# AnnSeidel/genometools

Hardware: AMD Instinct MI355X
Metric: Gbp/s ESA build (suf+lcp+bwt), 3 Gbp DNA, 1/2/4/8 MI355X; bit-exact vs CPU (higher is better)
Workload: dtype u64; 1 GPU; human-like DNA (2% N, 24 seqs, repeats) n=3000000000 seed=43 -suf -lcp -bwt (BASELINE.json configs[2]); parallelism=1 device, pair_suffixes=341032298, tied_suffixes=390540711, refine_rounds=9, maxbranchdepth=8256

## Files before the change

### genometools_amd/csrc/esa_engine.hip

```cpp
#include <stdarg.h>
#include <stdlib.h>
#include <chrono>
#include <type_traits>
#include <utility>
#include <vector>
#include "../../include/gtamd_esa.h"
#include "esa_prims.h"
#include "esa_devutil.h"
#include "esa_own.h"

static thread_local char g_err[1024] = "";
void gtamd_set_error(const char *fmt, ...) {
  va_list ap;
  va_start(ap, fmt);
  vsnprintf(g_err, sizeof g_err, fmt, ap);
  va_end(ap);
}
extern "C" const char *gtamd_esa_last_error(void) { return g_err; }

extern "C" int gtamd_device_count(void) {
  GTAMD_ABI_BEGIN
  int n = 0;
  if (hipGetDeviceCount(&n) != hipSuccess) return 0;
  return n;
// ... 2434 lines not shown
    return e != nullptr && e[0] == c;
  };
  if (const char *e = getenv("GTAMD_MSD")) sw.msd = e[0] == '1';
  sw.msd_part_off = flag("GTAMD_MSD", '0');
  if (const char *e = getenv("GTAMD_MSD_CBITS")) {
    const int v = atoi(e);
    if (v >= 0 && v <= 8) sw.msd_cbits = v;
  }
  if (const char *e = getenv("GTAMD_MSD_BIG_MAX")) {
    const long v = atol(e);
    if (v >= MS_TILE && v <= (long) MSD_BIG_MAX) sw.msd_big_max = (u32) v;
  }
  sw.msd_radix = flag("GTAMD_MSD_RADIX", '1');
  if (const char *e = getenv("GTAMD_MSD_PACK")) sw.msd_pack = atoi(e) != 0;
  if (const char *e = getenv("GTAMD_MSD_PACK_CAP")) {
    const long v = atol(e);
    if (v >= 1024 && v <= (long) MD_CAP) sw.msd_pack_cap = (u32) v;
  }
  if (const char *e = getenv("GTAMD_MSD_BIN_LIMIT")) {
    const long v = atol(e);
    if (v >= 2 && v <= 4096) sw.msd_bin_limit = (u32) v;
  }
  sw.fused_pass0 = !flag("GTAMD_FUSED_PASS0", '0');
  sw.force_wide = flag("GTAMD_FORCE_WIDE", '1');
  sw.no_pairs = flag("GTAMD_NO_PAIRS", '1');
  sw.no_small_groups = flag("GTAMD_NO_SMALL_GROUPS", '1');
  if (const char *e = getenv("GTAMD_APPLY_EARLY")) sw.apply_early = atoi(e);
  if (sw.apply_early < 0 || sw.apply_early > 2) sw.apply_early = 0;
  if (const char *e = getenv("GTAMD_APPLY_WGS")) {
    const long v = atol(e);
    if (v >= 64 && v <= (1 << 22)) sw.apply_wgs = (u64) v;
    sw.apply_wgs_given = true;
  }
  if (const char *e = getenv("GTAMD_RANK_WINDOW_BITS")) {
    const int v = atoi(e);
    if (v >= 2 && v <= RW_BITS) sw.rank_window_bits = v;
  }
  sw.rank_all_windows = flag("GTAMD_RANK_ALL_WINDOWS", '1');
  sw.win_filter_global = flag("GTAMD_WIN_FILTER_LDS", '0');
  if (const char *e = getenv("GTAMD_PAIR_CHUNK")) {
    const int v = atoi(e);
    if (v >= 4 && v <= 1024) sw.pair_chunk = v;
  }
  if (const char *e = getenv("GTAMD_ROUND_STRIDE")) {
    const int v = atoi(e);
    if (v >= RT_STRIDE_MIN && v <= RT_TILE) sw.round_stride = (u32) v;
  }
  sw.debug = getenv("GTAMD_DEBUG") != nullptr;
  return sw;
}

struct gtamd_esa_ctx {
  int device = 0;
  u32 sigma = 0;
  int bits = 0;
  u64 max_n = 0, n = 0, N = 0;
  int readmode = 0;
  Stream st, st2;
  Event ev_sorted, ev_emitted, ev_applied;
  DevBuf tb_own, sp_own;
  Text text = {};
  bool have_text = false;
  DevBuf k0, k1, v0, v1;
  DevBuf isa_tmp;
  DevBuf rws;
  DevBuf msd;
  DevBuf suf, lcp, bwt;
  DevBuf tiebits, tiebits2;
  DevBuf arena;
  DevBuf arena_p;
  DevBuf xrecv;
  DevBuf winbuf;
  DevBuf lcpfull_buf;
  DevBuf partws;
  DevBuf posw;
  Dev<u64> llv;
  u64 llv_pairs = 0;
  Dev<u32> bck;
  u64 bck_codes = 0, bck_special = 0, bck_dist = 0;
  Dev<Stats> d_stats;
  Pinned<Stats> h_stats;
  Pinned<u32> h_counts;
  Pinned<u32> h_hist;
  u32 user_prefixlength = 0;
  u32 part = 0, numparts = 1;
  gtamd_allgather_fn comm_allgather = nullptr;
  gtamd_alltoallv_fn comm_alltoallv = nullptr;
  void (*comm_abort)(void *) = nullptr;
  void *comm_abort_user = nullptr;
  void *comm_user = nullptr;
  u64 NL = 0, index_offset = 0;
  Dev<u32> d_parthist;
  Dev<u8> d_owner;
  Dev<u32> d_counts;
  u32 want = 0;
  bool ran = false;
  gtamd_esa_stats stats = {};
  gtamd_esa_timing timing = {};
  u64 alloc_bytes = 0;
  float alloc_ms = 0;
  Event ev[8];
  Event ev_scatter[2 * 16];
};

enum TimingEvent {
  EV_START,
  EV_KEYS,
  EV_SORTED,
  EV_TIEBITS,
  EV_REFINE_BEGIN,
  EV_REFINE_END,
  EV_DONE
};

static int ensure_buf(gtamd_esa_ctx *c, DevBuf &b, u64 bytes, const char *what) {
  if (bytes <= b.bytes) return 0;
  HIP_TRY(hipStreamSynchronize(c->st));
  HIP_TRY(hipStreamSynchronize(c->st2));
  const auto t0 = std::chrono::steady_clock::now();
  c->alloc_bytes -= b.bytes;
  b.reset();
  bytes = (bytes + 255) & ~255ull;
  const hipError_t me = b.alloc(bytes);
  c->alloc_ms += std::chrono::duration<float, std::milli>(std::chrono::steady_clock::now() - t0).count();
  if (me != hipSuccess) {
    (void) hipGetLastError();
    size_t mfree = 0, mtotal = 0;
    (void) hipMemGetInfo(&mfree, &mtotal);
    gtamd_set_error("cannot allocate %llu bytes of device memory for %s: the "
                    "context holds %llu bytes already, %llu of the device's %llu "
                    "are free",
                    (unsigned long long) bytes, what,
                    (unsigned long long) c->alloc_bytes, (unsigned long long) mfree,
                    (unsigned long long) mtotal);
    return -1;
  }
  c->alloc_bytes += bytes;
  return 0;
}

extern "C" void gtamd_esa_destroy(gtamd_esa_ctx *c) {
  if (c == nullptr) return;
  (void) hipSetDevice(c->device);
  if (c->st != nullptr) (void) hipStreamSynchronize(c->st);
  if (c->st2 != nullptr) (void) hipStreamSynchronize(c->st2);
  delete c;
}

static u64 max_positions(int bits) {
  const int spare = bits == 2 ? Key<2>::SPARE_BITS : Key<5>::SPARE_BITS;
  const int total = 32 + spare > 40 ? 40 : 32 + spare;
  return 1ull << total;
}

static int create_resources(gtamd_esa_ctx *c) {
  HIP_TRY(hipSetDevice(c->device));
  HIP_TRY(create(c->st, hipStreamNonBlocking));
  HIP_TRY(create(c->st2, hipStreamNonBlocking));
  HIP_TRY(create(c->ev_sorted, hipEventDisableTiming));
  HIP_TRY(create(c->ev_emitted, hipEventDisableTiming));
  HIP_TRY(create(c->ev_applied, hipEventDisableTiming));
  HIP_TRY(c->d_stats.alloc(sizeof(Stats)));
  HIP_TRY(c->h_stats.alloc(sizeof(Stats)));
  HIP_TRY(c->h_counts.alloc(4 * DEST_MAXPARTS * 4));
  HIP_TRY(c->h_hist.alloc(PART_BINS * 4));
  HIP_TRY(c->d_parthist.alloc(PART_BINS * 4));
  HIP_TRY(c->d_owner.alloc(PART_BINS));
  HIP_TRY(c->d_counts.alloc(4 * DEST_MAXPARTS * 4));
  for (Event &e : c->ev) HIP_TRY(create(e));
  for (Event &e : c->ev_scatter) HIP_TRY(create(e));
  return 0;
}

extern "C" gtamd_esa_ctx *gtamd_esa_create(int device, uint64_t max_n,
                                           uint32_t numofchars) {
  GTAMD_ABI_BEGIN
  if (gtamd_device_count() <= device || device < 0) {
    gtamd_set_error("no HIP device %d available (this library has no CPU "
                    "fallback)", device);
    return nullptr;
  }
  if (numofchars < 2 || numofchars > 28) {
    gtamd_set_error("alphabet size %u not supported (2..28)", numofchars);
    return nullptr;
  }
  const int bits = numofchars <= 4 ? 2 : 5;
  if (max_n + 1 >= max_positions(bits) - 4096) {
    gtamd_set_error("sequence of %llu symbols exceeds the position range of "
                    "this engine (%llu)", (unsigned long long) max_n,
                    (unsigned long long) max_positions(bits));
    return nullptr;
  }
  gtamd_esa_ctx *c = new gtamd_esa_ctx();
  c->device = device;
  c->sigma = numofchars;
// ... 243 lines not shown
  return 0;
}
template <typename F>
static int dest_place(gtamd_esa_ctx *c, const F &f, u64 m, const u8 *dest, const u32 *boff) {
  if (m == 0) return 0;
  const u64 nb = div_up(m, 256);
  k_dest_place<F><<<(u32) nb, 256, 0, c->st>>>(f, m, c->numparts, nb, dest, boff);
  HIP_TRY(hipGetLastError());
  return 0;
}
static u64 dest_words(u32 R, u64 m) { return (u64) R * div_up(m ? m : 1, 256) + 16; }

template <int BITS>
static int build_bcktab(gtamd_esa_ctx *c, const u64 *skey, const u32 *spos, u64 NL, u32 k,
                        hipStream_t st) {
  u64 codes = 1, special = 1, dist = 0, pw = 1;
  for (u32 j = 0; j < k; j++) {
    if (codes > (1ull << 31) / c->sigma) {
      gtamd_set_error("bucket table for prefixlength %u over %u letters is too "
                      "large", k, c->sigma);
      return -1;
    }
    codes *= c->sigma;
  }
  for (u32 j = 0; j + 1 < k; j++) special *= c->sigma;
  for (u32 j = 1; j + 1 < k; j++) { pw *= c->sigma; dist += pw; }
  const u64 total = codes + 1 + special + dist;
  HIP_TRY(c->bck.alloc(total * 4));
  HIP_TRY(hipMemsetAsync(c->bck, 0, total * 4, st));
  if (NL > 0) {
    k_bck_count<BITS><<<(u32) div_up(NL, 256), 256, 0, st>>>(
        skey, NL, k, c->sigma, c->bck, c->bck + codes + 1,
        c->bck + codes + 1 + special, c->text, spos);
    HIP_TRY(hipGetLastError());
  }
  u32 *ws = c->rws.as<u32>();
  Dev<u32> own;
  if (scan_workspace_words(codes + 1) * 4 > c->rws.bytes) {
    HIP_TRY(own.alloc(scan_workspace_words(codes + 1) * 4));
    ws = own;
  }
  TRY(scan_u32(SCAN_SUM, c->bck, c->bck, codes + 1, false, ws, st));
  c->bck_codes = codes; c->bck_special = special; c->bck_dist = dist;
  return 0;
}

static u64 rws_words_for(u64 cap) {
  return radix_workspace_words(cap) + 10 * (div_up(cap, 64) + 64) +
         scan_workspace_words(div_up(cap, 64)) + 64;
}
static int ensure_workspace(gtamd_esa_ctx *c, u64 cap, u32 want, bool dist) {
  const u64 pad = cap + 8;
  TRY(ensure_buf(c, c->k0, pad * 8, "sort keys"));
  TRY(ensure_buf(c, c->k1, pad * 8, "sort keys"));
  TRY(ensure_buf(c, c->v0, pad * 4, "sort values"));
  TRY(ensure_buf(c, c->v1, pad * 4, "sort values"));
  TRY(ensure_buf(c, c->rws, rws_words_for(cap) * 4, "the radix workspace"));
  TRY(ensure_buf(c, c->tiebits, (div_up(cap, 64) + 2) * 8, "the tie bitmap"));
  if (want & GTAMD_WANT_SUF) TRY(ensure_buf(c, c->suf, pad * 8, "the suffix table"));
  if (want & GTAMD_WANT_LCP) TRY(ensure_buf(c, c->lcp, pad, "the lcp table"));
  if (want & GTAMD_WANT_BWT) TRY(ensure_buf(c, c->bwt, pad, "the bwt table"));
  if (dist) TRY(ensure_buf(c, c->isa_tmp, pad * 8, "the exchange scratch"));
  return 0;
}

static int msd_cbits_max(u64 N) {
  const int c = bits_for(N > 1 ? N - 1 : 1) - 24;
  return c < 0 ? 0 : (c > 8 ? 8 : c);
}
static int msd_choose_cbits(u64 N, int cmax, const float *penalty) {
  int best = cmax;
  float best_cost = 0.0f;
  for (int k = 1; k >= 0; k--) {
    const int c = cmax - 2 + k;
    if (c < 6) continue;
    const float gain = k == 1 ? 0.17f : 0.57f;
    const float cost = (penalty[k] - penalty[2]) / (float) N - gain;
    if (cost < best_cost) { best = c; best_cost = cost; }
  }
  return best;
}
struct MsdWs {
  u32 *hist, *scanws, *tcnt, *tfirst, *dtcnt, *dtfirst, *startA, *startB, *F, *scan2, *counters,
      *biglist, *giantlist, *crowdlist, *bndA;
  MsTile *desc;
  MdTile *dtiles;
  u64 *firstkey, *lastkey;
  u32 rows, tilesB_ub, tilesC_ub, tilesD_ub;
  u64 nf;
};
static u64 msd_carve(u64 N, int cb, u8 *base, MsdWs *w) {
  const u32 ntA = (u32) div_up(N, MS_TILE);
  w->tilesB_ub = ntA + 256;
  w->tilesC_ub = ntA + MSD_PARENTS;
  w->tilesD_ub = (u32) (2 * div_up(N, MS_TILE)) + MSD_PARENTS + 8;
  w->rows = w->tilesC_ub + 2;
  w->nf = (u64) MSD_PARENTS << cb;
  Bump b;
  b.base = base;
  b.off = 0;
  w->hist = b.take<u32>((u64) w->rows * 256);
  w->scanws = b.take<u32>(radix_rows_workspace_words(w->rows));
  w->desc = b.take<MsTile>(w->tilesC_ub);
  w->tcnt = b.take<u32>(MSD_PARENTS + 8);
  w->tfirst = b.take<u32>(MSD_PARENTS + 8);
  w->dtcnt = b.take<u32>(MSD_PARENTS + 8);
  w->dtfirst = b.take<u32>(MSD_PARENTS + 8);
  w->startA = b.take<u32>(256 + 8);
  w->bndA = b.take<u32>(256 * MSD_BLOCKS);
  w->startB = b.take<u32>(MSD_PARENTS + 8);
  w->F = b.take<u32>(w->nf + 8);
  w->scan2 = b.take<u32>(scan_workspace_words(w->nf + 1) + 64);
  w->counters = b.take<u32>(16);
  w->dtiles = b.take<MdTile>(w->tilesD_ub);
  w->firstkey = b.take<u64>(w->tilesD_ub);
  w->lastkey = b.take<u64>(w->tilesD_ub);
  w->biglist = b.take<u32>(w->tilesD_ub);
  w->crowdlist = b.take<u32>(w->tilesD_ub);
  w->giantlist = b.take<u32>((u64) (N / MS_TILE) + 8);
  return b.off + 256;
}

static int msd_level_prepare(gtamd_esa_ctx *c, const MsdWs &w, const u32 *pstart, u32 np, int cb,
                             u32 tiles_ub, const u32 *kin, const u64 *ein, u32 *cstart) {
  hipStream_t st = c->st;
  k_msd_tilecount<<<(np + 1 + 255) / 256, 256, 0, st>>>(pstart, 0, np, (u32) MS_TILE, w.tcnt);
  HIP_TRY(hipGetLastError());
  TRY(scan_u32(SCAN_SUM, w.tcnt, w.tfirst, (u64) np + 1, false, w.scan2, st));
  k_msd_tiledesc<<<(tiles_ub + 255) / 256, 256, 0, st>>>(pstart, w.tfirst, np, tiles_ub, w.desc);
  HIP_TRY(hipGetLastError());
  if (ein != nullptr)
    k_msd_hist_lvl<u64><<<tiles_ub + 1, MS_THREADS, 0, st>>>(ein, w.desc, tiles_ub, 32 - cb, w.hist);
  else
    k_msd_hist_lvl<u32><<<tiles_ub + 1, MS_THREADS, 0, st>>>(kin, w.desc, tiles_ub, 32 - cb, w.hist);
  HIP_TRY(hipGetLastError());
  TRY(radix_scan_tile_rows(w.hist, tiles_ub + 1, w.scanws, st));
  const u64 nchild = (u64) np << cb;
  k_msd_tot<<<(u32) div_up(nchild + 1, 256), 256, 0, st>>>(w.hist, w.tfirst, np, cb, cstart);
  HIP_TRY(hipGetLastError());
  TRY(scan_u32(SCAN_SUM, cstart, cstart, nchild + 1, false, w.scan2, st));
  return 0;
}

struct MsdPartSrc {
  const u64 *ck;
  const u32 *cp32;
  u64 index_offset;
  const unsigned long long *prev_key;
  int has_prev;
};
template <int FMT>
static int msd_sort_emit(gtamd_esa_ctx *c, const Switches &sw, u32 want, u32 prefixlength, u64 N,
                         u64 density_n, const MsdPartSrc *src, u32 **sa_out,
                         u64 **fkey, u32 **fval, u64 *local_entries) {
  hipStream_t st = c->st;
  const int cmax = msd_cbits_max(density_n);
  int cb = sw.msd_cbits >= 0 ? sw.msd_cbits : cmax;
  MsdWs w;
  const u64 bytes = msd_carve(N, cb > cmax ? cb : cmax, nullptr, &w);
  TRY(ensure_buf(c, c->msd, bytes, "the tables of the first sort"));
  (void) msd_carve(N, cb > cmax ? cb : cmax, c->msd.as<u8>(), &w);
  const u32 ntA = (u32) div_up(N, MS_TILE);
  const u32 last_valid = (u32) (N - (u64) (ntA - 1) * MS_TILE);
  const u64 pad = N + 8;
  u32 *ka = c->k0.as<u32>(), *pa = c->v0.as<u32>();
  u32 *kb = c->k1.as<u32>(), *pb = c->v1.as<u32>();
  u8 *xa = c->k1.as<u8>() + pad * 4;
  u64 *ea = c->k0.as<u64>();
  const bool wide = src == nullptr;
  const int lbits = msd_block_bits(N);
  if (src != nullptr)
    k_msd_hist_a_keys<<<ntA, MS_THREADS, 0, st>>>(src->ck, N, w.hist);
  else if (FMT == 1)
    k_msd_hist_a5<<<ntA, MS_THREADS, 0, st>>>(c->text, N, w.hist);
  else
    k_msd_hist_a<<<ntA, MS_THREADS, 0, st>>>(c->text, N, w.hist);
  HIP_TRY(hipGetLastError());
  TRY(radix_scan_tile_rows(w.hist, ntA, w.scanws, st));
  k_msd_starts_a<<<wide ? MSD_BLOCKS : 1, 256, 0, st>>>(w.hist, (u32) N, ntA, lbits, w.startA,
                                                         wide ? w.bndA : nullptr);
  HIP_TRY(hipGetLastError());
  if (src != nullptr)
    k_msd_scatter_a<1><<<((ntA + 7u) >> 3) * 8u, MS_THREADS, 0, st>>>(
        c->text, N, last_valid, w.hist, ntA, src->ck, src->cp32, ka, xa, pa, nullptr);
  else if (FMT == 1)
    k_msd_scatter_a<2><<<((ntA + 7u) >> 3) * 8u, MS_THREADS, 0, st>>>(
        c->text, N, last_valid, w.hist, ntA, nullptr, nullptr, nullptr, nullptr, nullptr, ea);
  else
    k_msd_scatter_a<0><<<((ntA + 7u) >> 3) * 8u, MS_THREADS, 0, st>>>(
        c->text, N, last_valid, w.hist, ntA, nullptr, nullptr, nullptr, nullptr, nullptr, ea);
  HIP_TRY(hipGetLastError());
  HIP_TRY(hipEventRecord(c->ev[EV_KEYS], st));
  TRY(msd_level_prepare(c, w, w.startA, 256, 8, w.tilesB_ub, ka, wide ? ea : nullptr, w.startB));
  if (wide)
    k_msd_scatter_lvl<1, true><<<((w.tilesB_ub + 7u) >> 3) * 8u, MS_THREADS, 0, st>>>(
        nullptr, nullptr, nullptr, ea, w.bndA, lbits, w.desc, w.tilesB_ub, w.hist, w.tfirst,
        w.startB, 8, 24, kb, pb);
  else
    k_msd_scatter_lvl<1, false><<<((w.tilesB_ub + 7u) >> 3) * 8u, MS_THREADS, 0, st>>>(
        ka, xa, pa, nullptr, nullptr, 0, w.desc, w.tilesB_ub, w.hist, w.tfirst, w.startB, 8, 24,
        kb, pb);
  HIP_TRY(hipGetLastError());
  if (sw.msd_cbits < 0 && cmax >= 1) {
    float *d_exp = reinterpret_cast<float *>(w.counters);
    float *h_exp = c->h_counts.as<float>();
    HIP_TRY(hipMemsetAsync(d_exp, 0, 16, st));
    k_msd_skew<<<MSD_PARENTS / 256, 256, 0, st>>>(w.startB, cmax, d_exp);
    HIP_TRY(hipGetLastError());
    HIP_TRY(hipMemcpyAsync(h_exp, d_exp, 12, hipMemcpyDeviceToHost, st));
    HIP_TRY(hipStreamSynchronize(st));
    cb = msd_choose_cbits(N, cmax, h_exp);
  }
  w.nf = (u64) MSD_PARENTS << cb;
  u32 *kf = kb, *pf = pb, *ko = ka, *po = pa;
  const u32 *F = w.startB;
  if (cb > 0) {
    TRY(msd_level_prepare(c, w, w.startB, MSD_PARENTS, cb, w.tilesC_ub, kb, nullptr, w.F));
    F = w.F;
    kf = ka; pf = pa; ko = kb; po = pb;
  }
  HIP_TRY(hipMemsetAsync(w.counters, 0, 64, st));
  const u32 pack_cap = sw.msd_pack_cap;
  const bool packed = sw.msd_pack;
  if (packed) {
    k_msd_pack<false><<<(MSD_PARENTS + 1 + 255) / 256, 256, 0, st>>>(F, cb, nullptr, pack_cap, w.dtcnt, nullptr,
                                                                nullptr, nullptr, nullptr, 0);
    HIP_TRY(hipGetLastError());
    TRY(scan_u32(SCAN_SUM, w.dtcnt, w.dtfirst, (u64) MSD_PARENTS + 1, false, w.scan2, st));
    k_msd_pack<true><<<(MSD_PARENTS + 1 + 255) / 256, 256, 0, st>>>(F, cb, w.dtfirst, pack_cap, nullptr, w.dtiles,
                                                               w.biglist, w.giantlist, w.counters,
                                                               sw.msd_big_max);
    HIP_TRY(hipGetLastError());
  } else {
  k_msd_tilecount<<<(MSD_PARENTS + 1 + 255) / 256, 256, 0, st>>>(F, cb, MSD_PARENTS, MSD_STRIDE,
                                                               w.dtcnt);
  HIP_TRY(hipGetLastError());
  TRY(scan_u32(SCAN_SUM, w.dtcnt, w.dtfirst, (u64) MSD_PARENTS + 1, false, w.scan2, st));
  k_msd_dtiles<<<(w.tilesD_ub + 255) / 256, 256, 0, st>>>(F, cb, w.dtfirst, w.tilesD_ub, w.dtiles,
                                                        w.biglist, w.giantlist, w.crowdlist,
                                                        w.counters, sw.msd_big_max);
  HIP_TRY(hipGetLastError());
  }
  u32 *hc = c->h_counts;
  HIP_TRY(hipMemcpyAsync(hc, w.counters, 16, hipMemcpyDeviceToHost, st));
  HIP_TRY(hipMemcpyAsync(hc + 4, w.dtfirst + MSD_PARENTS, 4, hipMemcpyDeviceToHost, st));
  HIP_TRY(hipStreamSynchronize(st));
  const u32 nbig = hc[0], maxrun = hc[1], nbigentries = hc[2], ngiant = hc[3], ntD = hc[4];
  char dpre[32] = "";
  if (src != nullptr) snprintf(dpre, sizeof dpre, "part %u: ", c->part);
  if (sw.debug) {
    fprintf(stderr, "gtamd: %smsd sort: %d bits at level C, %u runs, %u big (largest %u, %u entries "
            "in all), %u giant\n", dpre, cb, ntD, nbig, maxrun, nbigentries, ngiant);
    std::vector<MdTile> dt(ntD);
    if (ntD > 0)
      HIP_TRY(hipMemcpy(dt.data(), w.dtiles, (size_t) ntD * sizeof(MdTile), hipMemcpyDeviceToHost));
    u32 largest = 0;
    for (const MdTile &d : dt) largest = d.end - d.begin > largest ? d.end - d.begin : largest;
    fprintf(stderr, "gtamd: %smsd level D: packed=%d pack_cap=%u tiles=%u largest=%u\n", dpre,
            (int) packed, pack_cap, ntD, largest);
  }
  std::vector<MdTile> giants(ngiant);
  std::vector<u32> giant_t(ngiant);
  if (ngiant > 0) {
    HIP_TRY(hipMemcpy(giant_t.data(), w.giantlist, (size_t) ngiant * 4, hipMemcpyDeviceToHost));
    for (u32 i = 0; i < ngiant; i++)
      HIP_TRY(hipMemcpy(&giants[i], w.dtiles + giant_t[i], sizeof(MdTile), hipMemcpyDeviceToHost));
  }
  if (cb > 0) {
    k_msd_scatter_lvl<2, false><<<((w.tilesC_ub + 7u) >> 3) * 8u, MS_THREADS, 0, st>>>(
        kb, nullptr, pb, nullptr, nullptr, 0, w.desc, w.tilesC_ub, w.hist, w.tfirst, w.F, cb,
        32 - cb, ka, pa);
    HIP_TRY(hipGetLastError());
  }
  MsdOut o;
  o.suf = (want & GTAMD_WANT_SUF) ? c->suf.as<u64>() : nullptr;
  o.lcp = (want & GTAMD_WANT_LCP) ? c->lcp.as<u8>() : nullptr;
  o.bwt = (want & GTAMD_WANT_BWT) ? c->bwt.as<u8>() : nullptr;
  o.sa = pf;
  o.tiebits = c->tiebits.as<u64>();
  o.firstkey = w.firstkey;
  o.lastkey = w.lastkey;
  o.stats = c->d_stats;
  o.prefixlength = prefixlength;
  o.index_offset = src != nullptr ? src->index_offset : 0;
  o.val_is_index = src != nullptr && src->cp32 == nullptr;
  if (o.val_is_index) o.suf = nullptr;
  HIP_TRY(hipMemsetAsync(o.tiebits, 0, (div_up(N, 64) + 2) * 8, st));
  if (ntD > 0) {
    HIP_TRY(hipEventRecord(c->ev_scatter[0], st));
    const int force_radix = sw.msd_radix ? 1 : 0;
    k_msd_local<FMT><<<stride_grid(ntD), MS_THREADS, 0, st>>>(kf, pf, w.dtiles, ntD, cb,
                                                        force_radix, sw.msd_bin_limit,
                                                        w.crowdlist, w.counters, o);
    HIP_TRY(hipEventRecord(c->ev_scatter[1], st));
    HIP_TRY(hipGetLastError());
    k_msd_local_radix<FMT><<<ntD < 2048u ? ntD : 2048u, MS_THREADS, 0, st>>>(kf, pf, w.dtiles,
                                                                        w.crowdlist, w.counters,
                                                                        cb, o);
    HIP_TRY(hipGetLastError());
    if (sw.debug) {
      HIP_TRY(hipMemcpyAsync(hc + 6, w.counters + 4, 4, hipMemcpyDeviceToHost, st));
      HIP_TRY(hipStreamSynchronize(st));
      fprintf(stderr, "gtamd: %smsd local: radix_runs=%u force_radix=%d bin_limit=%u\n", dpre, hc[6],
              force_radix, sw.msd_bin_limit);
    }
  }
  if (nbig > 0) {
    k_msd_big<FMT><<<nbig < 2048u ? nbig : 2048u, MS_THREADS, 0, st>>>(kf, pf, ko, po, w.dtiles,
                                                                w.biglist, w.counters, cb, o);
    HIP_TRY(hipGetLastError());
  }
  for (u32 i = 0; i < ngiant; i++) {
    const MdTile g = giants[i];
    const u64 cnt = g.end - g.begin;
    const int shifts[4] = {FMT == 1 ? 8 : 3, FMT == 1 ? 14 : 11, FMT == 1 ? 20 : 19, FMT == 1 ? 26 : 27};
    const int widths[4] = {FMT == 1 ? 6 : 8, FMT == 1 ? 6 : 8, FMT == 1 ? 6 : 8, FMT == 1 ? 6 : 5};
    int nev = 0;
    TRY(radix_sort_pairs<u32, u32>(kf + g.begin, pf + g.begin, ko + g.begin, po + g.begin, cnt,
                                   shifts, widths, 4, c->rws.as<u32>(), st, nullptr, &nev));
    k_msd_emit_run<FMT><<<(u32) div_up(cnt, MS_TILE), MS_THREADS, 0, st>>>(kf, pf, giant_t[i], g.begin,
                                                                     (u32) cnt, g.s16, o);
    HIP_TRY(hipGetLastError());
  }
  if (ntD > 0) {
    k_msd_seams<FMT><<<(ntD + 255) / 256, 256, 0, st>>>(w.dtiles, ntD, src != nullptr ? src->prev_key : nullptr,
                                                   src != nullptr ? src->has_prev : 0, o);
    HIP_TRY(hipGetLastError());
  }
  *sa_out = pf;
  *fkey = reinterpret_cast<u64 *>(ko);
  *fval = po;
  *local_entries = N - nbigentries;
  c->stats.msd_big_entries = nbigentries;
  return 0;
}

static int passes_for(int from, int to, int *ps, int *pw) {
  int cnt = 0;
  for (int b = from; b < to; b += 8) {
    ps[cnt] = b;
    pw[cnt] = to - b < 8 ? to - b : 8;
    cnt++;
  }
  return cnt;
}

template <typename T>
static std::vector<u32> range_cuts(const T *bins, u32 R) {
  u64 nsamp = 0;
  for (int b = 0; b < PART_BINS; b++) nsamp += bins[b];
  std::vector<u32> cut(R + 1);
  cut[0] = 0;
  cut[R] = PART_BINS;
  u64 run = 0;
  u32 b = 0;
  for (u32 r = 1; r < R; r++) {
    const u64 target = (u64) (((unsigned __int128) nsamp * r) / R);
    while (b < (u32) PART_BINS && run < target) run += bins[b++];
    cut[r] = b;
  }
  return cut;
}

enum Reduce { RED_SUM, RED_AND, RED_OR, RED_MAX };
static int allgather_word(gtamd_esa_ctx *c, int failed, Reduce op, u64 *word) {
  std::vector<u64> all(c->numparts);
  TRY(comm_allgather(c, failed, word, all.data(), 8));
  u64 v = all[0];
  for (u32 r = 1; r < c->numparts; r++)
    switch (op) {
      case RED_SUM: v += all[r]; break;
      case RED_AND: v &= all[r]; break;
      case RED_OR: v |= all[r]; break;
      case RED_MAX: v = all[r] > v ? all[r] : v; break;
    }
  *word = v;
  return 0;
}

static void set_slice_error(u64 NL) {
  gtamd_set_error("slice of %llu entries exceeds the 32-bit index range of one "
                  "part: use more parts", (unsigned long long) NL);
}

struct WinFilterTies {
  const u64 *tiebits2;
  const u32 *carry;
  const u64 *swp;
};
template <typename Q>
static int launch_win_filter(gtamd_esa_ctx *c, const Switches &sw, const Q *sa, u64 NL, int wb,
                             const u32 *sel, u64 nww, u32 nww_global, const u32 *pref,
                             const WinFilterTies &t, Q *fpos, u32 *fhead, u64 cap, u64 windows) {
  hipStream_t st = c->st;
  const bool wf_lds = (nww + 4) * 5 <= WF_LDS_MAX && !sw.win_filter_global;
  if (sw.debug)
    fprintf(stderr, "gtamd: part %u: win filter: bitmap=%s windows=%llu\n", c->part,
            wf_lds ? "lds" : "global", (unsigned long long) windows);
  const u32 grid = (u32) div_up(NL, WF_SPAN * WF_ITER);
  if (wf_lds) {
    HIP_TRY(hipFuncSetAttribute(reinterpret_cast<const void *>(&k_win_filter<Q, true>),
                                hipFuncAttributeMaxDynamicSharedMemorySize,
// ... 1589 lines not shown
```

### genometools_amd/csrc/esa_msd.h

```cpp
#pragma once
#include "esa_msd_blocks.h"

constexpr int MS_TILE = 4096;
constexpr int MS_THREADS = 512;
constexpr int MS_WAVES = MS_THREADS / 64;
constexpr int MS_ITEMS = MS_TILE / MS_THREADS;
constexpr int MS_WCHUNK = MS_ITEMS * 64;
constexpr int MS_PAD = 520;
constexpr u32 MSD_PARENTS = 65536;
constexpr u32 MSD_STRIDE = 3328;
constexpr int MD_ITEMS = 8;
constexpr u32 MD_CAP = MD_ITEMS * MS_THREADS;
constexpr u32 MSD_BIG_MAX = 1u << 19;

struct MsTile {
  u32 start;
  u32 segvalid;
};
struct MdTile {
  u32 begin, end;
  u32 s16;
  u32 pad;
};
struct MsdOut {
// ... 144 lines not shown
#pragma unroll
  for (int g = 0; g < KP_PER; g++) {
    const u64 win = g ? (a_hi << (2 * g)) | (a_lo >> (64 - 2 * g)) : a_hi;
    const u64 s = (S >> g) & ((1ull << SYMS) - 1ull);
    const int d = s ? __ffsll((unsigned long long) s) - 1 : SYMS;
    if (d == 0) {
      key[g] = (~0ull << K::DSHIFT) | pay;
    } else {
      u64 pre = win >> K::LOW_BITS;
      u32 dc = 0;
      if (d < SYMS) {
        pre |= (1ull << (2 * (SYMS - d))) - 1ull;
        dc = (u32) (SYMS - d);
      }
      key[g] = (pre << K::LOW_BITS) | ((u64) dc << K::DSHIFT) | pay;
    }
    const u32 c = (u32) (win >> 62);
    pay = (c < 2u && (s & 1ull)) ? ((c & 1u) ? P::SEP : P::WILD) : c;
  }
}

template <int NB>
__device__ __forceinline__ void ms_match(u32 d, u32 &intra, u32 &group) {
  u32 mlo = ~0u, mhi = ~0u;
#pragma unroll
  for (int b = 0; b < NB; b++) {
    u32 sx = (u32) ((int) (d << (31 - b)) >> 31);
    asm volatile("" : "+v"(sx));
    const u64 bal = __ballot(sx != 0);
    mlo = __builtin_amdgcn_bitop3_b32(mlo, (u32) bal, sx, 0x90);
    mhi = __builtin_amdgcn_bitop3_b32(mhi, (u32) (bal >> 32), sx, 0x90);
  }
  intra = __builtin_amdgcn_mbcnt_hi(mhi, __builtin_amdgcn_mbcnt_lo(mlo, 0u));
  group = (u32) __popc(mlo) + (u32) __popc(mhi);
}

typedef __attribute__((address_space(3))) volatile u16 ms_vu16;

__device__ __forceinline__ void lds_barrier() {
  asm volatile("s_waitcnt lgkmcnt(0)\n\ts_barrier" ::: "memory");
}
__device__ __forceinline__ u32 ms_scan_excl(u32 v, u32 *lds8) {
  const int lane = threadIdx.x & 63, w = threadIdx.x >> 6;
  const u32 inc = wave_scan_incl<SCAN_SUM>(v);
  if (lane == 63) lds8[w] = inc;
  lds_barrier();
  u32 carry = 0;
#pragma unroll
  for (int i = 0; i < MS_WAVES; i++) {
    const u32 x = lds8[i];
    if (i < w) carry += x;
  }
  lds_barrier();
  return carry + (inc - v);
}

__global__ __launch_bounds__(MS_THREADS) void k_msd_hist_a5(Text t, u64 N, u32 *__restrict__ hist) {
  __shared__ u32 h[MS_WAVES][256];
  const int tid = threadIdx.x, w = tid >> 6;
  for (int i = tid; i < MS_WAVES * 256; i += MS_THREADS) (&h[0][0])[i] = 0;
  __syncthreads();
  const u64 p0 = (u64) blockIdx.x * MS_TILE + (u64) tid * KP_PER;
  if (p0 < N) {
    const int npos = N - p0 < KP_PER ? (int) (N - p0) : KP_PER;
    u64 key[KP_PER];
    p5_keys8(t, p0, key);
#pragma unroll
    for (int g = 0; g < KP_PER; g++)
      if (g < npos) atomicAdd(&h[w][(u32) (key[g] >> 56)], 1u);
  }
  __syncthreads();
  if (tid < 256) {
    u32 c = 0;
#pragma unroll
    for (int i = 0; i < MS_WAVES; i++) c += h[i][tid];
    hist[(u64) blockIdx.x * 256 + tid] = c;
  }
}

__global__ __launch_bounds__(MS_THREADS) void k_msd_hist_a(Text t, u64 N,
                                                           u32 *__restrict__ hist) {
  __shared__ u32 h[MS_WAVES][256];
  const int tid = threadIdx.x, w = tid >> 6;
  for (int i = tid; i < MS_WAVES * 256; i += MS_THREADS) (&h[0][0])[i] = 0;
  __syncthreads();
  const u64 p0 = (u64) blockIdx.x * MS_TILE + (u64) tid * KP_PER;
  if (p0 < N) {
    const int npos = N - p0 < KP_PER ? (int) (N - p0) : KP_PER;
    u64 key[KP_PER];
    dna_keys8(t, p0, key);
#pragma unroll
    for (int g = 0; g < KP_PER; g++)
      if (g < npos) atomicAdd(&h[w][(u32) (key[g] >> 56)], 1u);
  }
  __syncthreads();
  if (tid < 256) {
    u32 c = 0;
#pragma unroll
    for (int i = 0; i < MS_WAVES; i++) c += h[i][tid];
    hist[(u64) blockIdx.x * 256 + tid] = c;
  }
}

struct DnaWin {
  u64 a_hi, a_lo;
  u64 S;
  u32 pay0;
};
__device__ __forceinline__ DnaWin dna_win(const Text &t, u64 p0) {
  using P = Pay<2>;
  DnaWin r;
  const u64 w = p0 >> 5;
  const int o = (int) (p0 & 31) * 2;
  const u64 hi = tb_word(t, w), lo = tb_word(t, w + 1);
  r.a_hi = o ? (hi << o) | (lo >> (64 - o)) : hi;
  r.a_lo = lo << o;
  const u64 sw = p0 >> 6;
  const int so = (int) (p0 & 63);
  const u64 s0 = sp_word(t, sw), s1 = sp_word(t, sw + 1);
  r.S = so ? (s0 >> so) | (s1 << (64 - so)) : s0;
  if (p0 == 0) {
    r.pay0 = P::UNDEF;
  } else {
    const u32 c = o ? (u32) (hi >> (64 - o)) & 3u : (u32) tb_word(t, w - 1) & 3u;
    const bool sp = c < 2u && (so ? (s0 >> (so - 1)) & 1ull : sp_word(t, sw - 1) >> 63);
    r.pay0 = sp ? ((c & 1u) ? P::SEP : P::WILD) : c;
  }
  return r;
}
__device__ __forceinline__ DnaWin dna_win_from(const Text &t, u64 p0, u64 hi, u64 lo, u64 s0, u64 s1) {
  using P = Pay<2>;
  DnaWin r;
  const u64 w = p0 >> 5;
  const int o = (int) (p0 & 31) * 2;
  r.a_hi = o ? (hi << o) | (lo >> (64 - o)) : hi;
  r.a_lo = lo << o;
  const u64 sw = p0 >> 6;
  const int so = (int) (p0 & 63);
  r.S = so ? (s0 >> so) | (s1 << (64 - so)) : s0;
  if (p0 == 0) {
    r.pay0 = P::UNDEF;
  } else {
    const u32 c = o ? (u32) (hi >> (64 - o)) & 3u : (u32) tb_word(t, w - 1) & 3u;
    const bool sp = c < 2u && (so ? (s0 >> (so - 1)) & 1ull : sp_word(t, sw - 1) >> 63);
    r.pay0 = sp ? ((c & 1u) ? P::SEP : P::WILD) : c;
  }
  return r;
}
__device__ __forceinline__ void dna_win_bins(const Text &t, u64 p0, u64 &a_hi, u32 &s14) {
  const u64 w = p0 >> 5;
  const int o = (int) (p0 & 31) * 2;
  const u64 hi = tb_word(t, w);
  a_hi = o ? (hi << o) | (tb_word(t, w + 1) >> (64 - o)) : hi;
  const u64 sw = p0 >> 6;
  const int so = (int) (p0 & 63);
  u64 S = sp_word(t, sw) >> so;
  if (so > 64 - 14) S |= sp_word(t, sw + 1) << (64 - so);
  s14 = (u32) S & 0x3FFFu;
}
__device__ __forceinline__ u32 dna_bins8_in_range(u64 a_hi, u32 s14, int npos, u32 lo, u32 width,
                                                  u32 &nbelow, u32 &mxbin) {
  u32 mask = 0;
  if (s14 == 0 && npos == KP_PER) {
#pragma unroll
    for (int g = 0; g < KP_PER; g++) {
      const u32 bin = (u32) ((a_hi << (2 * g)) >> (64 - PART_BITS));
      if (bin - lo < width) mask |= 1u << g;
      else if (bin < lo) { nbelow++; mxbin = bin > mxbin ? bin : mxbin; }
    }
    return mask;
  }
#pragma unroll
  for (int g = 0; g < KP_PER; g++) {
    if (g < npos) {
      u32 bin = (u32) ((a_hi << (2 * g)) >> (64 - PART_BITS));
      const u32 s7 = (s14 >> g) & 0x7Fu;
// ... 1178 lines not shown
        __syncthreads();
#pragma unroll
        for (int j = 0; j < MS_ITEMS; j++) {
          const u32 e = (u32) w * MS_WCHUNK + (u32) j * 64 + lane;
          const u32 d = e < valid ? (key[j] >> shift) & 255u : 255u;
          u32 intra, group;
          ms_match<8>(d, intra, group);
          const u32 old = cnt_w[d];
          if (intra == 0) cnt_w[d] = (u16) (old + group);
          rk[j] = ((old + intra) << 8) | d;
        }
        __syncthreads();
        {
          u32 c[MS_WAVES];
          u32 tot = 0;
          if (tid < 256) {
#pragma unroll
            for (int i = 0; i < MS_WAVES; i++) {
              c[i] = s_cnt[i * 256 + tid];
              tot += c[i];
            }
          }
          u32 all;
          u32 dbase = block_scan_excl<SCAN_SUM, MS_THREADS>(tot, &all, s_scan);
          if (tid < 256) {
            const u32 cur = s_cur[tid];
            s_obase[tid] = cur - dbase;
            s_cur[tid] = cur + tot - (tid == 255 ? (u32) MS_TILE - valid : 0u);
#pragma unroll
            for (int i = 0; i < MS_WAVES; i++) {
              s_cnt[i * 256 + tid] = (u16) dbase;
              dbase += c[i];
            }
          }
        }
        __syncthreads();
#pragma unroll
        for (int j = 0; j < MS_ITEMS; j++) {
          const u32 d = rk[j] & 255u;
          const u32 pos = (u32) cnt_w[d] + (rk[j] >> 8);
          s_key[pos] = key[j];
          s_val[pos] = val[j];
        }
        __syncthreads();
#pragma unroll
        for (int j = 0; j < MS_ITEMS; j++) {
          const u32 e = (u32) j * MS_THREADS + tid;
          if (e < valid) {
            const u32 k = s_key[e];
            const u32 g = s_obase[(k >> shift) & 255u] + e;
            dk[g] = k + base;
            dp[g] = s_val[e];
          }
        }
        __syncthreads();
      }
      u32 *x = sk; sk = dk; dk = x;
      x = sp; sp = dp; dp = x;
    }
    u32 prevkey = 0;
    for (u32 c0 = 0; c0 < cnt; c0 += (u32) MS_TILE) {
      const u32 valid = cnt - c0 < (u32) MS_TILE ? cnt - c0 : (u32) MS_TILE;
#pragma unroll
      for (int j = 0; j < MS_ITEMS; j++) {
        const u32 e = (u32) j * MS_THREADS + tid;
        if (e < valid) {
          s_key[e] = sk[c0 + e] - base;
          s_val[e] = sp[c0 + e];
        }
      }
      __syncthreads();
      if (tid == 0) {
        if (c0 == 0) o.firstkey[t] = msd_full<FMT>(td.s16, s_key[0] + base);
        if (c0 + valid == cnt) o.lastkey[t] = msd_full<FMT>(td.s16, s_key[valid - 1] + base);
      }
      const u32 lastk = s_key[valid - 1] + base;
      msd_emit<FMT>(s_key, s_val, valid, (u64) td.begin + c0, base, c0 > 0, prevkey, td.s16, o, s_bits, acc);
      prevkey = lastk;
    }
  }
  msd_acc_flush(acc, o.stats);
}

template <int FMT>
__global__ __launch_bounds__(MS_THREADS) void k_msd_emit_run(
    const u32 *__restrict__ kin, const u32 *__restrict__ pin, u32 t, u32 begin, u32 cnt, u32 s16,
    MsdOut o) {
  __shared__ u32 s_key[MS_TILE];
  __shared__ u32 s_val[MS_TILE];
  __shared__ u32 s_bits[(MS_TILE + 128) / 32];
  const int tid = threadIdx.x;
  MsdAcc acc;
  acc.sum = acc.ties = 0;
  acc.mx = 0;
  const u32 c0 = blockIdx.x * (u32) MS_TILE;
  const u32 valid = cnt - c0 < (u32) MS_TILE ? cnt - c0 : (u32) MS_TILE;
#pragma unroll
  for (int j = 0; j < MS_ITEMS; j++) {
    const u32 e = (u32) j * MS_THREADS + tid;
    if (e < valid) {
      s_key[e] = kin[(u64) begin + c0 + e];
      s_val[e] = pin[(u64) begin + c0 + e];
    }
  }
  __syncthreads();
  if (tid == 0) {
    if (c0 == 0) o.firstkey[t] = msd_full<FMT>(s16, s_key[0]);
    if (c0 + valid == cnt) o.lastkey[t] = msd_full<FMT>(s16, s_key[valid - 1]);
  }
  const u32 prevkey = c0 > 0 ? kin[(u64) begin + c0 - 1] : 0u;
  msd_emit<FMT>(s_key, s_val, valid, (u64) begin + c0, 0u, c0 > 0, prevkey, s16, o, s_bits, acc);
  msd_acc_flush(acc, o.stats);
}

template <int FMT>
__global__ __launch_bounds__(256) void k_msd_seams(const MdTile *__restrict__ tiles, u32 ntiles,
                                                   const unsigned long long *__restrict__ prev_key_p,
                                                   int has_prev, MsdOut o) {
  using K = Key<2>;
  const u32 t = blockIdx.x * 256u + threadIdx.x;
  MsdAcc acc;
  acc.sum = acc.ties = 0;
  acc.mx = 0;
  if (t < ntiles) {
    const MdTile td = tiles[t];
    if (td.end > td.begin && (td.begin > 0 || has_prev)) {
      u64 a = has_prev ? (u64) *prev_key_p : 0ull;
      if (td.begin > 0) {
        u32 u = t - 1;
        while (u > 0 && tiles[u].end == tiles[u].begin) u--;
        a = o.lastkey[u];
      }
      const u64 b = o.firstkey[t];
      u32 da, db, m;
      if (FMT == 1) {
        da = p5_letters(a >> 8); db = p5_letters(b >> 8);
        m = p5_common(a >> 8, b >> 8);
      } else {
        da = K::letters(a); db = K::letters(b);
        const u64 x = (a ^ b) >> K::LOW_BITS;
        m = x ? (u32) (__clzll((long long) x) - K::LOW_BITS) / 2u : (u32) K::SYMS;
      }
      u32 l = m < da ? m : da;
      l = l < db ? l : db;
      if (o.lcp != nullptr) o.lcp[td.begin] = (u8) l;
      acc.mx = l;
      if (db >= o.prefixlength) acc.sum = l;
    }
  }
  msd_acc_flush(acc, o.stats);
}
```

Before: 26.71 Gbp/s.

## Size giant-tile radix passes from the varying key bits; fast-path DNA histogram

Adds a kernel that ORs the XOR of each giant tile's keys against its first key, giving the set of key bits that actually vary. The host reads these masks back and picks the number, shift and width of the radix passes from that bit span, skipping the sort entirely when no bits vary, instead of always running four fixed passes. Separately, the level-A DNA histogram kernel now loads its text and special-character words before clearing shared memory, and takes a fast path that skips per-position special handling when a thread's window has no special characters. The cost is an extra scan over the giant tiles plus a host synchronisation before the giant sorts.

```diff
diff --git a/genometools_amd/csrc/esa_engine.hip b/genometools_amd/csrc/esa_engine.hip
--- a/genometools_amd/csrc/esa_engine.hip
+++ b/genometools_amd/csrc/esa_engine.hip
@@ -2540,6 +2540,7 @@
   Pinned<Stats> h_stats;
   Pinned<u32> h_counts;
   Pinned<u32> h_hist;
+  Pinned<u32> h_giant;
   u32 user_prefixlength = 0;
   u32 part = 0, numparts = 1;
   gtamd_allgather_fn comm_allgather = nullptr;
@@ -2568,7 +2569,8 @@
   EV_TIEBITS,
   EV_REFINE_BEGIN,
   EV_REFINE_END,
-  EV_DONE
+  EV_DONE,
+  EV_GIANT_BITS
 };
 
 static int ensure_buf(gtamd_esa_ctx *c, DevBuf &b, u64 bytes, const char *what) {
@@ -2978,7 +2980,7 @@
 }
 struct MsdWs {
   u32 *hist, *scanws, *tcnt, *tfirst, *dtcnt, *dtfirst, *startA, *startB, *F, *scan2, *counters,
-      *biglist, *giantlist, *crowdlist, *bndA;
+      *biglist, *giantlist, *giantbits, *crowdlist, *bndA;
   MsTile *desc;
   MdTile *dtiles;
   u64 *firstkey, *lastkey;
@@ -3014,6 +3016,7 @@
   w->biglist = b.take<u32>(w->tilesD_ub);
   w->crowdlist = b.take<u32>(w->tilesD_ub);
   w->giantlist = b.take<u32>((u64) (N / MS_TILE) + 8);
+  w->giantbits = b.take<u32>((u64) (N / MS_TILE) + 8);
   return b.off + 256;
 }
 
@@ -3036,6 +3039,22 @@
   HIP_TRY(hipGetLastError());
   TRY(scan_u32(SCAN_SUM, cstart, cstart, nchild + 1, false, w.scan2, st));
   return 0;
+}
+
+static int msd_giant_passes(u32 bits, int pb, int *shifts, int *widths) {
+  if (bits == 0) return 0;
+  int lo = pb + __builtin_ctz(bits);
+  const int hi = pb + 32 - __builtin_clz(bits);
+  int np = (hi - lo + 7) / 8;
+  np += np & 1;
+  int total = hi - lo > np ? hi - lo : np;
+  if (lo + total > 32) lo = 32 - total;
+  for (int i = 0, b = lo; i < np; i++) {
+    widths[i] = total / np + (i < total % np ? 1 : 0);
+    shifts[i] = b;
+    b += widths[i];
+  }
+  return np;
 }
 
 struct MsdPartSrc {
@@ -3168,6 +3187,15 @@
         32 - cb, ka, pa);
     HIP_TRY(hipGetLastError());
   }
+  if (ngiant > 0) {
+    HIP_TRY(c->h_giant.grow((u64) ngiant * 4));
+    HIP_TRY(hipMemsetAsync(w.giantbits, 0, (size_t) ngiant * 4, st));
+    k_msd_giant_bits<<<dim3(ngiant < 8u ? 2048u : 256u, ngiant < 65535u ? ngiant : 65535u), 256, 0, st>>>(
+        kf, w.dtiles, w.giantlist, ngiant, MsdFmt<FMT>::PB, w.giantbits);
+    HIP_TRY(hipGetLastError());
+    HIP_TRY(hipMemcpyAsync(c->h_giant, w.giantbits, (size_t) ngiant * 4, hipMemcpyDeviceToHost, st));
+    HIP_TRY(hipEventRecord(c->ev[EV_GIANT_BITS], st));
+  }
   MsdOut o;
   o.suf = (want & GTAMD_WANT_SUF) ? c->suf.as<u64>() : nullptr;
   o.lcp = (want & GTAMD_WANT_LCP) ? c->lcp.as<u8>() : nullptr;
@@ -3206,14 +3234,23 @@
                                                                 w.biglist, w.counters, cb, o);
     HIP_TRY(hipGetLastError());
   }
+  if (ngiant > 0) HIP_TRY(hipEventSynchronize(c->ev[EV_GIANT_BITS]));
   for (u32 i = 0; i < ngiant; i++) {
     const MdTile g = giants[i];
     const u64 cnt = g.end - g.begin;
-    const int shifts[4] = {FMT == 1 ? 8 : 3, FMT == 1 ? 14 : 11, FMT == 1 ? 20 : 19, FMT == 1 ? 26 : 27};
-    const int widths[4] = {FMT == 1 ? 6 : 8, FMT == 1 ? 6 : 8, FMT == 1 ? 6 : 8, FMT == 1 ? 6 : 5};
+    const u32 bits = c->h_giant[i];
+    int shifts[4], widths[4];
+    const int np = msd_giant_passes(bits, MsdFmt<FMT>::PB, shifts, widths);
+    if (sw.debug) {
+      char line[128];
+      snprintf(line, sizeof line, "gtamd: %smsd giant: entries=%llu bits=0x%x passes=%d\n", dpre,
+               (unsigned long long) cnt, bits, np);
+      fputs(line, stderr);
+    }
     int nev = 0;
-    TRY(radix_sort_pairs<u32, u32>(kf + g.begin, pf + g.begin, ko + g.begin, po + g.begin, cnt,
-                                   shifts, widths, 4, c->rws.as<u32>(), st, nullptr, &nev));
+    if (np > 0)
+      TRY(radix_sort_pairs<u32, u32>(kf + g.begin, pf + g.begin, ko + g.begin, po + g.begin, cnt,
+                                     shifts, widths, np, c->rws.as<u32>(), st, nullptr, &nev));
     k_msd_emit_run<FMT><<<(u32) div_up(cnt, MS_TILE), MS_THREADS, 0, st>>>(kf, pf, giant_t[i], g.begin,
                                                                      (u32) cnt, g.s16, o);
     HIP_TRY(hipGetLastError());
diff --git a/genometools_amd/csrc/esa_msd.h b/genometools_amd/csrc/esa_msd.h
--- a/genometools_amd/csrc/esa_msd.h
+++ b/genometools_amd/csrc/esa_msd.h
@@ -250,16 +250,37 @@
                                                            u32 *__restrict__ hist) {
   __shared__ u32 h[MS_WAVES][256];
   const int tid = threadIdx.x, w = tid >> 6;
+  const u64 p0 = (u64) blockIdx.x * MS_TILE + (u64) tid * KP_PER;
+  const int o = (int) (p0 & 31) * 2, so = (int) (p0 & 63);
+  u64 hi = 0, lo = 0, s0 = 0, s1 = 0;
+  if (p0 < N) {
+    hi = tb_word(t, p0 >> 5); lo = tb_word(t, (p0 >> 5) + 1);
+    s0 = sp_word(t, p0 >> 6); s1 = sp_word(t, (p0 >> 6) + 1);
+  }
   for (int i = tid; i < MS_WAVES * 256; i += MS_THREADS) (&h[0][0])[i] = 0;
   __syncthreads();
-  const u64 p0 = (u64) blockIdx.x * MS_TILE + (u64) tid * KP_PER;
   if (p0 < N) {
     const int npos = N - p0 < KP_PER ? (int) (N - p0) : KP_PER;
-    u64 key[KP_PER];
-    dna_keys8(t, p0, key);
-#pragma unroll
-    for (int g = 0; g < KP_PER; g++)
-      if (g < npos) atomicAdd(&h[w][(u32) (key[g] >> 56)], 1u);
+    const u64 a_hi = o ? (hi << o) | (lo >> (64 - o)) : hi;
+    const u64 S = so ? (s0 >> so) | (s1 << (64 - so)) : s0;
+    const u32 s11 = (u32) S & 0x7FFu;
+    if (s11 == 0 && npos == KP_PER) {
+#pragma unroll
+      for (int g = 0; g < KP_PER; g++) atomicAdd(&h[w][(u32) ((a_hi << (2 * g)) >> 56)], 1u);
+    } else {
+#pragma unroll
+      for (int g = 0; g < KP_PER; g++) {
+        if (g < npos) {
+          u32 d8 = (u32) ((a_hi << (2 * g)) >> 56);
+          const u32 s4 = (s11 >> g) & 0xFu;
+          if (s4) {
+            const int d = __ffs((int) s4) - 1;
+            d8 = d == 0 ? 255u : d8 | ((1u << (2 * (4 - d))) - 1u);
+          }
+          atomicAdd(&h[w][d8], 1u);
+        }
+      }
+    }
   }
   __syncthreads();
   if (tid < 256) {
@@ -1604,6 +1625,24 @@
   msd_acc_flush(acc, o.stats);
 }
 
+__global__ __launch_bounds__(256) void k_msd_giant_bits(const u32 *__restrict__ kin,
+                                                        const MdTile *__restrict__ tiles,
+                                                        const u32 *__restrict__ giantlist, u32 ngiant,
+                                                        int pb, u32 *__restrict__ bits) {
+  for (u32 gi = blockIdx.y; gi < ngiant; gi += gridDim.y) {
+    const MdTile td = tiles[giantlist[gi]];
+    const u32 first = kin[td.begin];
+    u32 x = 0;
+    for (u64 i = (u64) td.begin + blockIdx.x * 256u + threadIdx.x; i < (u64) td.end;
+         i += (u64) gridDim.x * 256u)
+      x |= kin[i] ^ first;
+    x >>= pb;
+#pragma unroll
+    for (int d = 32; d >= 1; d >>= 1) x |= __shfl_xor(x, d, 64);
+    if ((threadIdx.x & 63) == 0 && x != 0) atomicOr(&bits[gi], x);
+  }
+}
+
 template <int FMT>
 __global__ __launch_bounds__(MS_THREADS) void k_msd_emit_run(
     const u32 *__restrict__ kin, const u32 *__restrict__ pin, u32 t, u32 begin, u32 cnt, u32 s16,
```

Measured after the change: 26.03 Gbp/s. -2.5%, worse.
